# christianhbye/21cmVAE

Measured on AMD Instinct MI355X. Metric: emulated signals/sec (batched predict), higher is better.
Workload: dtype f16 (f32 accumulate)

## Files before the change

21cmvae_amd/_native.py:

```python
import ctypes as C
import os
import threading
import weakref

import numpy as np

HERE = os.path.dirname(os.path.abspath(__file__))
LIB_PATH = os.environ.get("V21_LIB") or os.path.join(HERE, "libv21.so")

PREC_F32, PREC_F16, PREC_BF16 = 0, 1, 2
PRECISIONS = {"f32": PREC_F32, "fp32": PREC_F32, "float32": PREC_F32,
              "f16": PREC_F16, "fp16": PREC_F16, "float16": PREC_F16,
              "bf16": PREC_BF16, "bfloat16": PREC_BF16}
ACT_LINEAR, ACT_RELU, ACT_GAUSS = 0, 1, 2
FWD_IN_TRANSFORM, FWD_OUT_TRANSFORM, FWD_FORCE_GENERIC, FWD_NO_SMALL, FWD_FORCE_CHAIN, FWD_FORCE_JIT = 1, 2, 4, 8, 16, 32
COMM_ID_BYTES = 128


class EngineUnavailable(RuntimeError):
    """libv21.so cannot be loaded or no MI355X is visible."""


class EngineError(RuntimeError):
    """A v21_* call returned a negative status."""
# ... 40 lines not shown


class SampleOut(C.Structure):
    _fields_ = [(k, C.c_void_p) for k in SAMPLE_OUTPUTS]


_P = C.c_void_p
_F = C.POINTER(C.c_float)
SIGNATURES = {
    "v21_last_error": (C.c_char_p, []),
    "v21_version": (C.c_int, []),
    "v21_device_count": (C.c_int, [C.POINTER(C.c_int)]),
    "v21_ctx_create": (C.c_int, [C.c_int, C.POINTER(_P)]),
    "v21_ctx_destroy": (C.c_int, [_P]),
    "v21_ctx_sync": (C.c_int, [_P]),
    "v21_ctx_set_stream": (C.c_int, [_P, _P]),
    "v21_ctx_get_stream": (C.c_int, [_P, C.POINTER(_P)]),
    "v21_malloc": (C.c_int, [_P, C.c_size_t, C.POINTER(_P)]),
    "v21_free": (C.c_int, [_P, _P]),
    "v21_memcpy_h2d": (C.c_int, [_P, _P, _P, C.c_size_t]),
    "v21_memcpy_d2h": (C.c_int, [_P, _P, _P, C.c_size_t]),
    "v21_memset": (C.c_int, [_P, _P, C.c_int, C.c_size_t]),
    "v21_event_create": (C.c_int, [_P, C.POINTER(_P)]),
    "v21_event_destroy": (C.c_int, [_P, _P]),
    "v21_event_record": (C.c_int, [_P, _P]),
    "v21_event_elapsed_ms": (C.c_int, [_P, _P, _P, C.POINTER(C.c_float)]),
    "v21_mlp_create": (C.c_int, [_P, C.c_int, C.POINTER(C.c_int), C.POINTER(C.c_int), C.POINTER(_P)]),
    "v21_mlp_destroy": (C.c_int, [_P]),
    "v21_mlp_num_params": (C.c_int, [_P, C.POINTER(C.c_size_t)]),
    "v21_mlp_set_weights": (C.c_int, [_P, _F, C.c_size_t]),
    "v21_mlp_get_weights": (C.c_int, [_P, _F, C.c_size_t]),
    "v21_mlp_set_input_transform": (C.c_int, [_P, C.POINTER(AffineIn)]),
    "v21_mlp_set_output_transform": (C.c_int, [_P, C.POINTER(AffineOut)]),
    "v21_mlp_has_fused": (C.c_int, [_P, C.c_int, C.POINTER(C.c_int)]),
    "v21_mlp_jit": (C.c_int, [_P, C.c_int, C.c_int, C.POINTER(C.c_int)]),
    "v21_jit_prebuild": (C.c_int, [C.c_int, C.POINTER(C.c_int), C.POINTER(C.c_int), C.c_int, C.c_char_p]),
    "v21_mlp_forward": (C.c_int, [_P, _P, C.c_int, C.c_int64, _F, C.c_int, C.c_int]),
    "v21_mlp_forward_dev": (C.c_int, [_P, _P, C.c_int64, C.c_int64, _P, C.c_int64, C.c_int, C.c_int]),
    "v21_trainer_create": (C.c_int, [_P, C.c_int, C.c_int, C.POINTER(_P)]),
    "v21_trainer_destroy": (C.c_int, [_P]),
    "v21_trainer_set_adam": (C.c_int, [_P, C.POINTER(Adam)]),
    "v21_trainer_set_lr": (C.c_int, [_P, C.c_float]),
    "v21_trainer_get_lr": (C.c_int, [_P, C.POINTER(C.c_float)]),
    "v21_trainer_set_data": (C.c_int, [_P, C.c_int, _F, _F, _F, C.c_int64]),
    "v21_trainer_run_epoch": (C.c_int, [_P, C.POINTER(C.c_int32), C.c_int, C.POINTER(C.c_double)]),
    "v21_trainer_eval": (C.c_int, [_P, C.c_int, C.c_int, C.POINTER(C.c_double)]),
    "v21_trainer_step_dev": (C.c_int, [_P, _P, _P, _P, C.c_int, C.c_int]),
    "v21_trainer_last_step_loss": (C.c_int, [_P, C.POINTER(C.c_double)]),
    "v21_trainer_get_state": (C.c_int, [_P, C.POINTER(C.c_int64), _F, _F, C.c_size_t]),
    "v21_trainer_set_state": (C.c_int, [_P, C.c_int64, _F, _F, C.c_size_t]),
    "v21_trainer_get_grad": (C.c_int, [_P, _F, C.c_size_t]),
    "v21_trainer_use_graph": (C.c_int, [_P, C.c_int]),
    "v21_debug_poison_lds": (C.c_int, [_P, C.c_uint32]),
    "v21_debug_check_chain_jobs": (C.c_int, [_P, C.c_longlong, C.c_longlong]),
    "v21_debug_trainer_counters": (C.c_int, [_P, C.POINTER(C.c_longlong)]),
    "v21_route_forward": (C.c_int, [C.c_int, C.POINTER(C.c_int), C.POINTER(C.c_int), C.c_int, C.c_int64, C.c_int, C.c_int, C.POINTER(C.c_int)]),
    "v21_route_train": (C.c_int, [C.c_int, C.POINTER(C.c_int), C.POINTER(C.c_int), C.c_int, C.c_int, C.c_int, C.c_int, C.c_int,
                                  C.POINTER(C.c_int), C.POINTER(C.c_int)]),
    "v21_trainer_jit": (C.c_int, [_P, C.c_int, C.POINTER(C.c_int)]),
    "v21_mlp_last_route": (C.c_int, [_P, C.POINTER(C.c_int), C.POINTER(C.c_longlong)]),
    "v21_mlp_jacobian": (C.c_int, [_P, _P, C.c_int, C.c_int64, _F, _F, C.c_int, C.c_int]),
    "v21_mlp_jacobian_dev": (C.c_int, [_P, _P, C.c_int64, C.c_int64, _P, C.c_int64, _P, C.c_int, C.c_int]),
    "v21_mlp_set_likelihood": (C.c_int, [_P, _F, _F, C.c_int32]),
    "v21_mlp_loglike": (C.c_int, [_P, _P, C.c_int, C.c_int64, _F, _F, C.c_int, C.c_int]),
    "v21_mlp_loglike_dev": (C.c_int, [_P, _P, C.c_int64, C.c_int64, _P, _P, C.c_int, C.c_int]),
    "v21_route_jacobian": (C.c_int, [C.c_int, C.POINTER(C.c_int), C.POINTER(C.c_int), C.c_int, C.c_int64, C.c_int, C.POINTER(C.c_int)]),
    "v21_mlp_last_jac_route": (C.c_int, [_P, C.POINTER(C.c_int), C.POINTER(C.c_longlong)]),
    "v21_mlp_fisher": (C.c_int, [_P, _P, C.c_int, C.c_int64, _F, _F, _F, C.c_int, C.c_int]),
    "v21_mlp_fisher_dev": (C.c_int, [_P, _P, C.c_int64, C.c_int64, _P, _P, _P, C.c_int, C.c_int]),
    "v21_mlp_fit": (C.c_int, [_P, _P, C.c_int, C.c_int64, _F, C.c_int64, C.POINTER(FitOpts), _P, _F, _F, _F, C.POINTER(C.c_int32),
                              C.c_int, C.c_int]),
    "v21_mlp_fit_dev": (C.c_int, [_P, _P, C.c_int64, C.c_int64, _P, C.c_int64, C.POINTER(FitOpts), _P, _P, _P, _P, _P, C.c_int, C.c_int]),
    "v21_mlp_sample": (C.c_int, [_P, _P, C.c_int, C.c_int64, _F, C.c_int64, C.POINTER(SampleOpts), _P, C.POINTER(SampleOut),
                                 C.c_int, C.c_int]),
    "v21_mlp_sample_dev": (C.c_int, [_P, _P, C.c_int64, C.c_int64, _P, C.c_int64, C.POINTER(SampleOpts), _P, C.POINTER(SampleOut),
                                     C.c_int, C.c_int]),
    "v21_nuisance_whiten": (C.c_int, [C.POINTER(C.c_double), _F, C.c_int32, C.c_int32, C.POINTER(C.c_double), C.POINTER(C.c_double)]),
    "v21_mlp_set_nuisance": (C.c_int, [_P, C.POINTER(C.c_double), C.c_int32, C.c_int32]),
    "v21_mlp_nuisance_info": (C.c_int, [_P, C.POINTER(C.c_int32)]),
    "v21_mlp_nuisance_coef": (C.c_int, [_P, _P, C.c_int, C.c_int64, C.POINTER(C.c_double), C.c_int, C.c_int]),
    "v21_trainer_last_route": (C.c_int, [_P, C.POINTER(C.c_int), C.POINTER(C.c_int), C.POINTER(C.c_longlong), C.POINTER(C.c_longlong)]),
    "v21_route_name": (C.c_char_p, [C.c_int, C.c_int]),
    "v21_trainer_get_data_dev": (C.c_int, [_P, C.c_int, C.POINTER(_P), C.POINTER(_P), C.POINTER(_P), C.POINTER(C.c_int64)]),
    "v21_debug_clock_probe_start": (C.c_int, [_P, C.c_double, C.c_double]),
    "v21_debug_forward_clocked": (C.c_int, [_P, _P, C.c_int64, C.c_int64, _P, C.c_int64, C.c_int, C.c_int, _P]),
    "v21_debug_clock_probe_read": (C.c_int, [_P, C.POINTER(C.c_double), C.POINTER(C.c_double), C.POINTER(C.c_double), C.POINTER(C.c_int)]),
    "v21_trainer_set_vae": (C.c_int, [_P, C.c_float, C.c_int, C.c_uint64]),
    "v21_trainer_enable_stamps": (C.c_int, [_P, C.c_int]),
    "v21_trainer_chain_stamps": (C.c_int, [_P, C.POINTER(C.c_uint64), C.c_int]),
    "v21_host_alloc": (C.c_int, [_P, C.c_size_t, C.POINTER(_P)]),
    "v21_host_free": (C.c_int, [_P, _P]),
    "v21_sweep_create": (C.c_int, [C.POINTER(_P), C.c_int, C.POINTER(_P)]),
    "v21_sweep_destroy": (C.c_int, [_P]),
    "v21_sweep_run_epoch": (C.c_int, [_P, C.POINTER(C.c_int32), C.c_int, C.POINTER(C.c_double)]),
    "v21_joint_create": (C.c_int, [_P, _P, C.c_int, C.POINTER(_P)]),
    "v21_joint_destroy": (C.c_int, [_P]),
    "v21_joint_run_epoch": (C.c_int, [_P, C.POINTER(C.c_int32), C.c_int, C.POINTER(C.c_double)]),
    "v21_joint_eval": (C.c_int, [_P, C.POINTER(C.c_double)]),
    "v21_comm_get_unique_id": (C.c_int, [_P, _P]),
    "v21_comm_init": (C.c_int, [_P, C.c_int, C.c_int, _P]),
    "v21_comm_init_host": (C.c_int, [_P, C.c_int, C.c_int, C.POINTER(CommHostOps)]),
    "v21_comm_destroy": (C.c_int, [_P]),
    "v21_comm_init_null": (C.c_int, [_P, C.c_int, C.c_int]),
    "v21_comm_set_buckets": (C.c_int, [_P, C.c_int]),
    "v21_trainer_phase_timing": (C.c_int, [_P, C.c_int, C.c_int]),
    "v21_trainer_phase_times": (C.c_int, [_P, C.POINTER(C.c_double), C.POINTER(C.c_int)]),
# ... 132 lines not shown
        h, self.h = self.h, None
        try:
            self._destroy(h)
        except Exception:
            pass
        parents, self._parents = self._parents, []
        for p in parents:
            p._children -= 1
            p._try_destroy()

    def __del__(self):
        try:
            if hasattr(self, "_finalized"):
                self._release()
        except Exception:
            pass


class Context:
    _default = {}

    def __init__(self, device=0):
        self.lib = load_library()
        n = C.c_int(0)
        st = self.lib.v21_device_count(C.byref(n))
        if st != 0 or n.value < 1:
            raise EngineUnavailable("no HIP device visible (v21_device_count -> %d, n=%d): the MI355X "
                                    "engine has no CPU fallback" % (st, n.value))
        h = _P()
        check(self.lib.v21_ctx_create(device, C.byref(h)))
        self.h, self.device = h, device
        self.lock = threading.Lock()
        self.nranks, self.rank = 1, 0
        self._host_ops = None
        self._pin_pool = {"free": [], "live": 0, "lock": threading.Lock()}

    @classmethod
    def default(cls, device=None):
        if device is None:
            device = int(os.environ.get("LOCAL_RANK", "0")) if os.environ.get("V21_DEVICE_FROM_RANK") else 0
        if device not in cls._default:
            cls._default[device] = cls(device)
        return cls._default[device]

    def sync(self):
        check(self.lib.v21_ctx_sync(self.h))

    def set_stream(self, hip_stream):
        check(self.lib.v21_ctx_set_stream(self.h, _P(hip_stream)))

    def poison_lds(self, pattern=0xFFFFFFFF):
        check(self.lib.v21_debug_poison_lds(self.h, pattern))

    def clock_probe_start(self, duration_ms, period_us=50.0):
        check(self.lib.v21_debug_clock_probe_start(self.h, float(duration_ms), float(period_us)))

    def clock_probe_read(self):
        a, b, c_, n = C.c_double(0), C.c_double(0), C.c_double(0), C.c_int(0)
        check(self.lib.v21_debug_clock_probe_read(self.h, C.byref(a), C.byref(b), C.byref(c_), C.byref(n)))
        return {"ghz_mean": a.value, "ghz_min": b.value, "ghz_max": c_.value, "samples": n.value}

    def memset(self, dptr, byte, nbytes):
        check(self.lib.v21_memset(self.h, _P(dptr), int(byte), int(nbytes)))

    def malloc(self, nbytes):
        p = _P()
        check(self.lib.v21_malloc(self.h, nbytes, C.byref(p)))
        return p.value

    PIN_MIN_BYTES = 8 << 20
    PIN_POOL_MAX = 4

    def pinned_empty(self, shape, dtype=np.float32):
        nbytes = int(np.prod(shape)) * np.dtype(dtype).itemsize
        if nbytes < self.PIN_MIN_BYTES:
            return None
        pool, ptr = self._pin_pool, None
        with pool["lock"]:
            for i, (p, cap) in enumerate(pool["free"]):
                if cap >= nbytes:
                    ptr, cap_ = pool["free"].pop(i)
                    break
            if ptr is None:
                if pool["live"] + len(pool["free"]) >= self.PIN_POOL_MAX:
                    if pool["free"]:
                        pool["free"].sort(key=lambda t: t[1])
                        q, _ = pool["free"].pop(0)
                        self.lib.v21_host_free(self.h, _P(q))
                    else:
                        return None
                hp = _P()
                if self.lib.v21_host_alloc(self.h, nbytes, C.byref(hp)) != 0:
                    return None
                ptr, cap_ = hp.value, nbytes
            pool["live"] += 1
        raw = (C.c_char * nbytes).from_address(ptr)
        arr = np.frombuffer(raw, dtype=dtype, count=int(np.prod(shape))).reshape(shape)

        def _back(pool=pool, ptr=ptr, cap=cap_):
            with pool["lock"]:
                pool["live"] -= 1
                pool["free"].append((ptr, cap))
        weakref.finalize(raw, _back)
        return arr

    def free(self, dptr):
# ... 586 lines not shown
```

21cmvae_amd/csrc/api_forward.hip:

```cpp
#include "api_internal.h"

namespace v21 {
#define V21_DECL(a)                                                      \
  hipError_t launch_fused_##a##_F32(const FusedArgs&, hipStream_t);      \
  hipError_t launch_fused_##a##_F16x2sp(const FusedArgs&, hipStream_t);  \
  hipError_t launch_fused_##a##_BF16x2sp(const FusedArgs&, hipStream_t);
V21_ARCH_LIST(V21_DECL)
#undef V21_DECL
hipError_t launch_fused_S1_F16x2spClk(const FusedArgs&, hipStream_t);
hipError_t launch_fused_S1_BF16x2spClk(const FusedArgs&, hipStream_t);
}

typedef hipError_t (*fused_launcher)(const FusedArgs&, hipStream_t);
struct FusedEntry {
  int L;
  const int* dims;
  const int* act;
  fused_launcher fn[3];
};
#define V21_ENTRY(a) \
  {Arch##a::L, Arch##a::dims, Arch##a::act, {launch_fused_##a##_F32, launch_fused_##a##_F16x2sp, launch_fused_##a##_BF16x2sp}},
static const FusedEntry g_fused[] = {V21_ARCH_LIST(V21_ENTRY)};
#undef V21_ENTRY

// ... 329 lines not shown
  hipError_t rt = hipSuccess;
  if (route == FWD_FUSED || route == FWD_FUSED_RT) {
    CHK(ensure_stream(m, precision));
    a.x = d_x; a.ldx = ldx; a.y = d_y; a.ldy = ldy; a.n_rows = n;
    a.stream = m->d_stream[precision];
    const bool tout = (flags & V21_FWD_OUT_TRANSFORM) != 0;
    a.out_std = tout ? m->out_std : 1.0f;
    a.out_mean_scale = tout ? 1.0f : 0.0f;
    a.in_transform = (flags & V21_FWD_IN_TRANSFORM) ? 1 : 0;
    if (a.in_transform) a.tin = m->tin;
#ifdef V21_FUSED_STAMP
    a.dbg = (unsigned long long*)(getenv("V21_FUSED_DBG_PTR") ? strtoull(getenv("V21_FUSED_DBG_PTR"), nullptr, 0) : 0ull);
#endif
  }
  if (route == FWD_FUSED_RT) {
    rt = v21::jit_launch(jk, m->ctx->device, a, m->ctx->stream);
    if (rt != hipSuccess) (void)hipGetLastError();
    if (rt != hipSuccess && !force_jit) { q.jit = 0; route = decide_forward(q); }
  }
  note_route(m, route);
  if (route == FWD_TABLE) return forward_chain(m, d_x, ldx, n, d_y, ldy, precision, flags);
  if (route == FWD_GENERIC) return forward_generic(m, d_x, ldx, n, d_y, ldy, precision, flags);
  if (route == FWD_FUSED_RT) {
    if (rt == hipSuccess) return V21_OK;
    std::string why;
    v21::jit_state(jk, &why);
    return fail(V21_ERR_UNSUPPORTED, "V21_FWD_FORCE_JIT: %s (%s)", why.c_str(), hipGetErrorString(rt));
  }
  if (m->clk_stamps) {
    a.dbg = m->clk_stamps;
    HIPCHK((precision == V21_PREC_F16 ? launch_fused_S1_F16x2spClk : launch_fused_S1_BF16x2spClk)(a, m->ctx->stream));
    return V21_OK;
  }
  HIPCHK(g_fused[m->fused_id].fn[precision](a, m->ctx->stream));
  return V21_OK;
}
extern "C" int v21_mlp_forward_dev(v21_mlp* m, const float* d_x, int64_t ldx, int64_t n, float* d_y, int64_t ldy,
                                   int precision, int flags) {
  CHK(fwd_args(m, d_x && d_y, true, n, ldx, ldy, V21_DTYPE_F32, precision, flags));
  return n == 0 ? V21_OK : forward_rows(m, d_x, ldx, n, d_y, ldy, precision, flags);
}
extern "C" int v21_debug_forward_clocked(v21_mlp* m, const float* d_x, int64_t ldx, int64_t n, float* d_y, int64_t ldy, int precision,
                                         int flags, unsigned long long* d_stamps) {
  if (!m || !d_stamps) return fail(V21_ERR_ARG, "null argument");
  if (m->fused_id < 0 || g_fused[m->fused_id].dims != ArchS1::dims || (precision != V21_PREC_F16 && precision != V21_PREC_BF16))
    return fail(V21_ERR_UNSUPPORTED, "clock-stamped kernels exist for the headline stack (archs.h S1) in f16 / bf16 only");
  if (flags & (V21_FWD_FORCE_GENERIC | V21_FWD_FORCE_CHAIN | V21_FWD_FORCE_JIT)) return fail(V21_ERR_ARG, "route flags do not apply");
  m->clk_stamps = d_stamps;
  const int r = v21_mlp_forward_dev(m, d_x, ldx, n, d_y, ldy, precision, flags | V21_FWD_NO_SMALL);
  m->clk_stamps = nullptr;
  return r;
}

extern "C" int v21_mlp_jit(v21_mlp* m, int precision, int wait_ms, int* status) {
  if (!m || !status) return fail(V21_ERR_ARG, "null argument");
  if (precision < 0 || precision > 2) return fail(V21_ERR_ARG, "precision %d unknown", precision);
  *status = -1;
  if (m->fused_id >= 0) { *status = 1; return V21_OK; }
  std::string why;
  if (!v21::jit_eligible(m->L, m->dims.data(), m->act.data(), &why)) return fail(V21_ERR_UNSUPPORTED, "no fused kernel for this stack: %s", why.c_str());
  v21::JitKernel* k = jit_kernel(m, precision);
  if (!k) return fail(V21_ERR_UNSUPPORTED, "run-time compilation is switched off (V21_JIT=0) and no cached kernel exists");
  int s = v21::jit_state(k);
  if (s == v21::JIT_COMPILING && wait_ms != 0) s = v21::jit_wait(k, wait_ms);
  *status = s;
  if (s == v21::JIT_FAILED) {
    v21::jit_state(k, &why);
    return fail(V21_ERR_UNSUPPORTED, "fused kernel of this stack: %s", why.c_str());
  }
  return V21_OK;
}
extern "C" int v21_jit_prebuild(int n_layers, const int* dims, const int* act, int precision, const char* dir) {
  if (!dims || !act) return fail(V21_ERR_ARG, "null argument");
  std::string why;
  if (v21::jit_prebuild(n_layers, dims, act, precision, dir, &why) != 0) return fail(V21_ERR_UNSUPPORTED, "%s", why.c_str());
  return V21_OK;
}

extern "C" int v21_mlp_forward(v21_mlp* m, const void* x, int x_dtype, int64_t n, float* y, int precision, int flags) {
  flags &= 0xFF;
  CHK(fwd_args(m, x && y, false, n, 0, 0, x_dtype, precision, flags));
  if (n == 0) return V21_OK;
  hipStream_t st = m->ctx->stream;
  const int din = m->dims[0], dout = m->dims[m->L];
  const long long chunk = 1 << 18;
  const size_t need = (size_t)std::min<long long>(n, chunk);
  CHK(m->d_xs.reserve(need * din));
  CHK(m->d_xs64.reserve(need * din));
  CHK(m->d_ys.reserve(need * dout));
  std::vector<float> tmp;
  const bool tin = (flags & V21_FWD_IN_TRANSFORM) != 0;
  auto host_value = [&](long long r, int j) -> float {
    const v21_affine_in& a = m->tin;
    if (x_dtype == V21_DTYPE_F64) {
      const double t = ((const double*)x)[r * din + j];
      if (!tin) return (float)t;
      return par_transform_f64(t, a.log_mask[j], a.zero_floor[j], a.lo[j], a.span[j]);
    }
    const float f = ((const float*)x)[r * din + j];
    if (!tin) return f;
    return par_transform_f32(f, a.log_mask[j], a.zero_floor[j], a.lo[j], a.span[j]);
  };
  const FwdQuery hq{m->L, m->dims.data(), m->act.data(), m->fused_id >= 0, 0, precision, (long long)n, flags & ~V21_FWD_IN_TRANSFORM, (long long)dout};
  if (decide_forward(hq) == FWD_SMALL && (!tin || din <= 8)) {
    const long long ldp = p16(din);
    CHK(m->d_xpad.reserve((size_t)(n + 2) * ldp));
// ... 184 lines not shown
```

21cmvae_amd/csrc/fused_fwd.h:

```cpp
#pragma once
#ifndef __HIPCC_RTC__
#include <hip/hip_runtime.h>
#endif

#include <type_traits>
#include <utility>

#include "../../include/v21_types.h"
#include "par_transform.h"

namespace v21 {

typedef float f32x16 __attribute__((ext_vector_type(16)));
typedef float f32x4 __attribute__((ext_vector_type(4)));
typedef _Float16 f16x8 __attribute__((ext_vector_type(8)));
typedef __bf16 bf16x8 __attribute__((ext_vector_type(8)));
typedef unsigned u32x4 __attribute__((ext_vector_type(4)));
typedef short i16x2 __attribute__((ext_vector_type(2)));
typedef float f32x2 __attribute__((ext_vector_type(2)));
typedef _Float16 f16x2 __attribute__((ext_vector_type(2)));
typedef __bf16 bf16x2 __attribute__((ext_vector_type(2)));

constexpr int kFragBytes = 1024;
constexpr int kWaves = 4;
// ... 201 lines not shown
      constexpr int I = decltype(i)::value;
      glds16(g + I * G::WAVES * kFragBytes, voff, s + I * G::WAVES * kFragBytes);
    });
  }
}

template <class G, int B, int I>
__device__ __forceinline__ void issue_piece(const unsigned char* gstream, unsigned char* smem,
                                            int wave, int lane) {
  if constexpr (B >= 0 && B < G::n_blocks()) {
    if constexpr (I < G::blk_glds(B)) {
      const unsigned char* g = gstream + (size_t)B * G::BLK * kFragBytes + I * G::WAVES * kFragBytes;
      const unsigned voff = wave * kFragBytes + lane * 16;
      const unsigned s = lds_addr(smem) + (B % G::RING) * G::BLK * kFragBytes + wave * kFragBytes +
                         I * G::WAVES * kFragBytes;
      glds16(g, voff, s);
    }
  }
}

template <class G, int CT, int D, int S, bool SPREAD>
__device__ __forceinline__ void ring_boundary(const unsigned char* gstream, unsigned char* smem,
                                              int wave, int lane, unsigned long long* g_dbg = nullptr) {
  constexpr int kBlkFrags = G::BLK, kRing = G::RING;
  if constexpr (S % kBlkFrags == 0 && S < G::padded()) {
    constexpr int B = S / kBlkFrags;
    constexpr int last_issued = (B + kRing - 3 > kRing - 1) ? B + kRing - 3 : kRing - 1;
    constexpr int GA = [] {
      int s = 0;
      for (int i = B + 1; i <= last_issued; ++i) s += G::blk_glds(i);
      return s;
    }();
    constexpr int S_issue = (B < kRing) ? 0 : (B - kRing + 2 + (SPREAD ? 1 : 0)) * kBlkFrags;
    constexpr int SA = G::stores_before_step(S, CT, D) - G::stores_before_step(S_issue, CT, D);
    constexpr int N = (GA + SA) > 63 ? 63 : (GA + SA);
#ifdef V21_FUSED_STAMP
    { unsigned long long t; asm volatile("s_memtime %0\n\ts_waitcnt lgkmcnt(0)" : "=s"(t)::"memory");
      ((unsigned long long*)(smem + G::RING * G::BLK * kFragBytes))[wave * 512 + 2 * B] = t; }
#endif
    wait_vmcnt_barrier<N>();
#ifdef V21_FUSED_STAMP
    { unsigned long long t; asm volatile("s_memtime %0\n\ts_waitcnt lgkmcnt(0)" : "=s"(t)::"memory");
      ((unsigned long long*)(smem + G::RING * G::BLK * kFragBytes))[wave * 512 + 2 * B + 1] = t; }
#endif
    if constexpr (B >= 2 && !SPREAD) issue_block<G, B + kRing - 2>(gstream, smem, wave, lane);
  }
}

template <class G, int F> __device__ __forceinline__ const unsigned char* frag_ptr(const unsigned char* smem, int lane) {
  constexpr int B = F / G::BLK;
  return smem + ((B % G::RING) * G::BLK + (F % G::BLK)) * kFragBytes + lane * 16;
}

template <class Arch, class P>
__global__ void __launch_bounds__(64 * P::WAVES, P::WPS) fused_fwd(const FusedArgs a) {
  constexpr int kWaves = P::WAVES;
  constexpr int kBlkFrags = P::BLK, kRing = P::RING, kFusedLds = fused_lds<P>();
  (void)kFusedLds;
  extern __shared__ __attribute__((aligned(16))) unsigned char smem[];
  using G = Geo<Arch, P>;
  using frag = typename P::frag;
  using Item = typename G::Item;
  constexpr int L = G::L, CT = P::CT, EPI = P::EPI, FPI = P::FPI, IPT = G::IPT;
  constexpr int KSM = G::ks_max();
#ifndef V21_FUSED_D
#define V21_FUSED_D 2
#endif
#ifndef V21_FUSED_SPREAD
#define V21_FUSED_SPREAD 0
#endif
  constexpr int D = P::DEPTH;
  constexpr bool SPREAD = (V21_FUSED_SPREAD != 0) || spread_of<P>::value;
  constexpr int TOTAL = G::total();
  constexpr int NOUT = G::dim(L);
  constexpr int NCH = CT * 8;
  static_assert(G::act(L - 1) == 0, "output layer must be linear");
  static_assert(G::nt_of(L - 1) == 1 || G::ks_of(L - 1) > P::DEPTH, "output layer: too few k-steps per tile for the aux double buffer");
  static_assert(D <= kBlkFrags, "read-ahead must stay within one block");

  const int lane = threadIdx.x & 63;
  const int wave = __builtin_amdgcn_readfirstlane(threadIdx.x >> 6);
  const int r = lane & 31, h = lane >> 5;
  unsigned long long clk_t0 = 0, clk_r0 = 0;
  if constexpr (clk_of<P>::value) {
    asm volatile("s_memtime %0\n\ts_memrealtime %1\n\ts_waitcnt lgkmcnt(0)" : "=s"(clk_t0), "=s"(clk_r0)::"memory");
  }
  const long long wg_row0 = (long long)blockIdx.x * (kWaves * CT * 32);
  const long long row0 = wg_row0 + wave * (CT * 32);

  unsigned bufA[CT][KSM][4], bufB[CT][KSM][4];

  {
    constexpr int K0 = G::dim(0);
    static_for<CT>([&](auto ct_) __attribute__((always_inline)) {
      constexpr int ct = decltype(ct_)::value;
      const long long row = row0 + ct * 32 + r;
      const bool ok = row < a.n_rows;
      const float* xr = a.x + (ok ? row : 0) * a.ldx;
      static_for<G::ks_of(0)>([&](auto ks_) __attribute__((always_inline)) {
        constexpr int ks = decltype(ks_)::value;
        float v[EPI];
        static_for<EPI>([&](auto e_) __attribute__((always_inline)) {
          constexpr int e = decltype(e_)::value;
          constexpr int f0 = FPI * ks + 8 * (e >> 2) + (e & 3);
          constexpr int f1 = f0 + 4;
          float t = 0.f;
          if constexpr (f0 < K0) {
            const bool valid = ok && (h == 0 || f1 < K0);
            if (valid) {
              t = xr[f0 + 4 * h];
              if (a.in_transform) {
                constexpr int g1 = f1 < 8 ? f1 : 7;
                constexpr int g0 = f0 < 8 ? f0 : 7;
                const double zf = h ? a.tin.zero_floor[g1] : a.tin.zero_floor[g0];
                const int lm = h ? a.tin.log_mask[g1] : a.tin.log_mask[g0];
                const double lo = h ? a.tin.lo[g1] : a.tin.lo[g0];
                const double sp = h ? a.tin.span[g1] : a.tin.span[g0];
                t = par_transform_f32(t, lm, zf, lo, sp);
              }
            }
          }
          v[e] = t;
        });
#pragma unroll
        for (int wd = 0; wd < 4; ++wd) {
          if constexpr (EPI == 8) bufA[ct][ks][wd] = P::pack2(v[2 * wd], v[2 * wd + 1]);
          else bufA[ct][ks][wd] = __builtin_bit_cast(unsigned, v[wd]);
        }
      });
    });
  }

  static_for<kRing>([&](auto b) __attribute__((always_inline)) {
    issue_block<G, decltype(b)::value>(a.stream, smem, wave, lane);
  });

  long long wg_rows = a.n_rows - wg_row0;
  if (wg_rows > kWaves * CT * 32) wg_rows = kWaves * CT * 32;
  if (wg_rows < 0) wg_rows = 0;
  const unsigned out_bytes = (unsigned)(wg_rows * a.ldy * 4);
  __amdgpu_buffer_rsrc_t orsrc =
      __builtin_amdgcn_make_buffer_rsrc((void*)(a.y + wg_row0 * a.ldy), 0, out_bytes, 0x00020000);
  const unsigned ldy_b = (unsigned)a.ldy * 4u;
  const unsigned ovoff = (unsigned)(wave * (CT * 32) + 4 * h) * ldy_b + (unsigned)r * 4u;

  frag q[D + 1];
  f32x16 auxb[2];
  f32x16 acc[2][CT];

  auto epilogue_chunk = [&](auto g_, auto c_) __attribute__((always_inline)) {
    constexpr int GT = decltype(g_)::value;
    constexpr int c = decltype(c_)::value;
    constexpr Item t = G::tile_at(GT);
    constexpr int l = t.l, nt = t.nt;
    constexpr int ct = c / 8, pr = c % 8;
    if constexpr (l < L - 1) {
      constexpr int item = IPT * nt + (2 * pr) / EPI, e0 = (2 * pr) % EPI;
      if constexpr (item < G::ks_of(l + 1)) {
        auto& out = (l & 1) ? bufA : bufB;
        const float x0 = acc[GT & 1][ct][2 * pr], x1 = acc[GT & 1][ct][2 * pr + 1];
        if constexpr (EPI == 8) {
          unsigned w = P::pack2(x0, x1);
          if constexpr (G::act(l) != 0) {
            const i16x2 z = {0, 0};
            w = __builtin_bit_cast(unsigned, __builtin_elementwise_max(__builtin_bit_cast(i16x2, w), z));
          }
          out[ct][item][e0 / 2] = w;
        } else {
          int b0 = __builtin_bit_cast(int, x0), b1 = __builtin_bit_cast(int, x1);
          if constexpr (G::act(l) != 0) { b0 = max(b0, 0); b1 = max(b1, 0); }
          out[ct][item][e0] = (unsigned)b0;
          out[ct][item][e0 + 1] = (unsigned)b1;
        }
      }
    } else {
      const float obias = auxb[GT & 1][0], omean = auxb[GT & 1][1] * a.out_mean_scale;
      unsigned voff = ovoff + (unsigned)(32 * nt) * 4u;
      if (32 * nt + r >= NOUT) voff = 0xFFFFFFF0u;
#pragma unroll
      for (int u = 0; u < 2; ++u) {
        const int i = 2 * pr + u;
        const unsigned soff = (unsigned)(ct * 32 + (i & 3) + 8 * (i >> 2)) * ldy_b;
        float y;
        if constexpr (EPI == 8) {
          y = __builtin_fmaf(acc[GT & 1][ct][i], a.out_std, __builtin_fmaf(obias, a.out_std, omean));
        } else {
          y = (acc[GT & 1][ct][i] + obias) * a.out_std + omean;
        }
// ... 52 lines not shown
        constexpr int GP = GT > 0 ? GT - 1 : 0;
        constexpr int CPK = G::chunks_per_kstep(GP, NCH);
        constexpr bool whole_first = (GT > 0) && (G::spread_limit(GP) == 0);
        if constexpr (whole_first && it.ks == 0) {
          epilogue_range(std::integral_constant<int, GP>{}, std::integral_constant<int, 0>{},
                         std::integral_constant<int, NCH>{});
        }
#ifdef V21_FUSED_STAMP
        if constexpr (it.ks == 0) {
          unsigned long long t; asm volatile("s_memtime %0\n\ts_waitcnt lgkmcnt(0)" : "=s"(t)::"memory");
          ((unsigned long long*)(smem + kFusedLds))[wave * 512 + 128 + GT] = t; }
#endif
        auto& in = (it.l & 1) ? bufB : bufA;
        const frag w = q[C % (D + 1)];
#pragma unroll
        for (int ct = 0; ct < CT; ++ct) {
          f32x16 c0;
          if constexpr (it.ks == 0) {
            if constexpr (it.l < L - 1) c0 = auxb[GT & 1];
            else
#pragma unroll
              for (int i = 0; i < 16; ++i) c0[i] = 0.f;
          } else {
            c0 = acc[GT & 1][ct];
          }
          acc[GT & 1][ct] = P::template mfma<(it.l == L - 1)>(w, operand(in, ct, it.ks), c0);
        }
        if constexpr (GT > 0 && !whole_first) {
          constexpr int lo = it.ks * CPK < NCH ? it.ks * CPK : NCH;
          constexpr int hi = (it.ks + 1) * CPK < NCH ? (it.ks + 1) * CPK : NCH;
          epilogue_range(std::integral_constant<int, GP>{}, std::integral_constant<int, lo>{},
                         std::integral_constant<int, hi>{});
        }
      }
    }
  });
  epilogue_range(std::integral_constant<int, G::n_tiles() - 1>{}, std::integral_constant<int, 0>{},
                 std::integral_constant<int, NCH>{});
  if constexpr (clk_of<P>::value) {
    unsigned long long t1, r1;
    unsigned xcc, hwid;
    asm volatile("s_memtime %0\n\ts_memrealtime %1\n\ts_getreg_b32 %2, hwreg(HW_REG_XCC_ID)\n\ts_getreg_b32 %3, hwreg(HW_REG_HW_ID)\n\ts_waitcnt lgkmcnt(0)"
                 : "=s"(t1), "=s"(r1), "=s"(xcc), "=s"(hwid)::"memory");
    if (a.dbg && wave == 0 && lane == 0) {
      unsigned long long* gd = a.dbg + (size_t)blockIdx.x * 5;
      gd[0] = clk_t0; gd[1] = clk_r0; gd[2] = t1; gd[3] = r1; gd[4] = (unsigned long long)(xcc & 0xF) | ((unsigned long long)hwid << 8);
    }
  }
#ifdef V21_FUSED_STAMP
  if (a.dbg) {
    unsigned long long t; asm volatile("s_memtime %0\n\ts_waitcnt lgkmcnt(0)" : "=s"(t)::"memory");
    unsigned long long* sd = (unsigned long long*)(smem + kFusedLds) + wave * 512;
    sd[127] = t;
    __builtin_amdgcn_s_waitcnt(0xC07F);
    unsigned long long* gd = a.dbg + ((size_t)blockIdx.x * kWaves + wave) * 512;
#pragma unroll
    for (int k = 0; k < 8; ++k) gd[64 * k + lane] = sd[64 * k + lane];
  }
#endif
}

}
```

21cmvae_amd/csrc/par_transform.h:

```cpp
#pragma once
#ifndef __HIPCC_RTC__
#include <hip/hip_runtime.h>
#endif

#include "../../include/v21_types.h"

namespace v21 {
__host__ __device__ __forceinline__ float par_transform_f32(float x, int lm, double zf, double lo, double span) {
  if (zf > 0.0 && x == 0.f) x = (float)zf;
  double t = (double)x;
  if (lm) t = (double)(float)log10(t);
  t -= lo; t /= span; t *= 2.0; t -= 1.0;
  return (float)t;
}
__host__ __device__ __forceinline__ float par_transform_f64(double t, int lm, double zf, double lo, double span) {
  if (zf > 0.0 && t == 0.0) t = zf;
  if (lm) t = log10(t);
  t -= lo; t /= span; t *= 2.0; t -= 1.0;
  return (float)t;
}
}
```

include/v21.h:

```cpp
#ifndef V21_H
#define V21_H

#include <stddef.h>
#include <stdint.h>

#ifdef __cplusplus
extern "C" {
#endif

typedef struct v21_ctx v21_ctx;
typedef struct v21_mlp v21_mlp;
typedef struct v21_trainer v21_trainer;

enum {
  V21_OK = 0,
  V21_ERR_ARG = -1,
  V21_ERR_HIP = -2,
  V21_ERR_UNSUPPORTED = -3,
  V21_ERR_STATE = -4,
  V21_ERR_COMM = -5
};

enum { V21_PREC_F32 = 0, V21_PREC_F16 = 1, V21_PREC_BF16 = 2 };
enum { V21_ACT_LINEAR = 0, V21_ACT_RELU = 1, V21_ACT_GAUSS = 2 };
// ... 64 lines not shown
int v21_route_jacobian(int n_layers, const int* dims, const int* act, int precision, int64_t n, int flags, int* route);
int v21_mlp_last_jac_route(v21_mlp* mlp, int* route, long long counts[4]);

int v21_mlp_fisher(v21_mlp* mlp, const void* x, int x_dtype, int64_t n, float* fisher, float* lnl, float* grad, int precision, int flags);
int v21_mlp_fisher_dev(v21_mlp* mlp, const float* d_x, int64_t ldx, int64_t n, float* d_fisher, float* d_lnl, float* d_grad,
                       int precision, int flags);
int v21_mlp_fit(v21_mlp* mlp, const void* x0, int x_dtype, int64_t n, const float* data, int64_t n_data, const v21_fit_opts* opts,
                void* x_hat, float* lnl, float* lnl_start, float* fisher, int32_t* status, int precision, int flags);
int v21_mlp_fit_dev(v21_mlp* mlp, const float* d_x0, int64_t ldx, int64_t n, const float* d_data, int64_t n_data,
                    const v21_fit_opts* opts, float* d_x_hat, float* d_lnl, float* d_lnl_start, float* d_fisher, int32_t* d_status,
                    int precision, int flags);

int v21_mlp_sample(v21_mlp* mlp, const void* x0, int x_dtype, int64_t n, const float* data, int64_t n_data, const v21_sample_opts* opts,
                   const double* eps_start, const v21_sample_out* out, int precision, int flags);
int v21_mlp_sample_dev(v21_mlp* mlp, const float* d_x0, int64_t ldx, int64_t n, const float* d_data, int64_t n_data,
                       const v21_sample_opts* opts, const double* d_eps_start, const v21_sample_out* out, int precision, int flags);

int v21_nuisance_whiten(const double* basis, const float* inv_var, int32_t n_modes, int32_t out_dim, double* q, double* r);
int v21_mlp_set_nuisance(v21_mlp* mlp, const double* basis, int32_t n_modes, int32_t out_dim);
int v21_mlp_nuisance_info(v21_mlp* mlp, int32_t* n_modes);
int v21_mlp_nuisance_coef(v21_mlp* mlp, const void* x, int x_dtype, int64_t n, double* coef, int precision, int flags);

typedef struct {
  float lr, beta1, beta2, eps;
} v21_adam;

int v21_trainer_create(v21_mlp* mlp, int precision, int max_batch, v21_trainer** out);
int v21_trainer_destroy(v21_trainer* tr);
int v21_trainer_set_adam(v21_trainer* tr, const v21_adam* cfg);
int v21_trainer_set_lr(v21_trainer* tr, float lr);
int v21_trainer_get_lr(v21_trainer* tr, float* lr);
int v21_trainer_set_data(v21_trainer* tr, int which , const float* x,
                         const float* y, const float* row_weight, int64_t n);
int v21_trainer_run_epoch(v21_trainer* tr, const int32_t* perm, int batch, double* loss);
int v21_trainer_eval(v21_trainer* tr, int which, int batch, double* loss);
int v21_trainer_get_data_dev(v21_trainer* tr, int which, const float** x, const float** y, const float** row_weight, int64_t* n);
int v21_trainer_step_dev(v21_trainer* tr, const float* d_x, const float* d_y,
                         const float* d_row_weight, int n_rows, int global_rows);
int v21_trainer_last_step_loss(v21_trainer* tr, double* loss);
int v21_trainer_get_state(v21_trainer* tr, int64_t* iter, float* m, float* v, size_t n);
int v21_trainer_set_state(v21_trainer* tr, int64_t iter, const float* m, const float* v,
                          size_t n);
int v21_trainer_get_grad(v21_trainer* tr, float* g, size_t n);
typedef struct v21_joint v21_joint;
int v21_joint_create(v21_trainer* ae, v21_trainer* em, int latent_layer, v21_joint** out);
int v21_joint_destroy(v21_joint* j);
int v21_joint_run_epoch(v21_joint* j, const int32_t* perm , int batch, double* losses );
int v21_joint_eval(v21_joint* j, double* losses );
int v21_trainer_use_graph(v21_trainer* tr, int enable);
int v21_debug_poison_lds(v21_ctx* ctx, uint32_t pattern);
int v21_debug_clock_probe_start(v21_ctx* ctx, double duration_ms, double period_us);
int v21_debug_forward_clocked(v21_mlp* mlp, const float* d_x, int64_t ldx, int64_t n, float* d_y, int64_t ldy, int precision,
                              int flags, unsigned long long* d_stamps);
int v21_debug_clock_probe_read(v21_ctx* ctx, double* ghz_mean, double* ghz_min, double* ghz_max, int* samples);
int v21_debug_check_chain_jobs(v21_trainer* tr, long long fw_bytes, long long bw_bytes);
int v21_route_forward(int n_layers, const int* dims, const int* act, int precision, int64_t n, int flags, int rt_ready, int* route);
int v21_route_train(int n_layers, const int* dims, const int* act, int precision, int max_batch, int rows, int nranks, int rt_ready, int* fwd, int* upd);
int v21_mlp_last_route(v21_mlp* mlp, int* route, long long counts[8]);
int v21_trainer_last_route(v21_trainer* tr, int* fwd, int* upd, long long fwd_counts[8], long long upd_counts[8]);
const char* v21_route_name(int kind, int route);
int v21_trainer_phase_timing(v21_trainer* tr, int steps, int cut);
int v21_trainer_phase_times(v21_trainer* tr, double* ms, int* steps);
int v21_debug_trainer_counters(v21_trainer* tr, long long out[4]);
int v21_trainer_enable_stamps(v21_trainer* tr, int enable);
int v21_trainer_chain_stamps(v21_trainer* tr, uint64_t* out, int n);
int v21_trainer_set_vae(v21_trainer* tr, float kl_weight, int sample, uint64_t seed);

typedef struct v21_sweep v21_sweep;
int v21_sweep_create(v21_trainer** trainers, int count, v21_sweep** out);
int v21_sweep_destroy(v21_sweep* sw);
int v21_sweep_run_epoch(v21_sweep* sw, const int32_t* perm, int batch, double* losses);

#define V21_COMM_ID_BYTES 128
typedef struct v21_comm_host_ops {
  void* user;
  int (*allreduce_sum_f32)(void* user, float* buf, size_t n);
  int (*reduce_scatter_sum_f32)(void* user, float* buf, size_t n_per);
  int (*allgather_f32)(void* user, float* buf, size_t n_per);
} v21_comm_host_ops;
int v21_comm_get_unique_id(v21_ctx* ctx, void* id );
int v21_comm_init(v21_ctx* ctx, int nranks, int rank, const void* id);
int v21_comm_init_host(v21_ctx* ctx, int nranks, int rank, const v21_comm_host_ops* ops);
int v21_comm_init_null(v21_ctx* ctx, int nranks, int rank);
int v21_comm_set_buckets(v21_ctx* ctx, int buckets);
int v21_comm_destroy(v21_ctx* ctx);
int v21_comm_set_sharded(v21_ctx* ctx, int on);
int v21_comm_info(v21_ctx* ctx, int* nranks, int* rank, int* transport);
int v21_comm_allreduce_f32(v21_ctx* ctx, float* d_buf, size_t n);
int v21_comm_reduce_scatter_f32(v21_ctx* ctx, float* d_buf, size_t n_per);
int v21_comm_allgather_f32(v21_ctx* ctx, float* d_buf, size_t n_per);

#ifdef __cplusplus
}
#endif
#endif
```

Baseline: 1.232 billion.

## Overlap weight prefetch with input loads and use fast parameter transform

The fused forward kernel now issues the weight-ring prefetch before the first-layer input loads and loads all input values up front, so the global loads overlap. The input parameter transform switches to a fast path that replaces the f64 log10 and division with a polynomial log plus Newton-refined reciprocal. A correctness check falls back to the exact routine when rounding is ambiguous. A debug comparison kernel and clock-stamp hooks are added to validate bit-exactness and profile the kernel head. This costs extra registers for the preloaded inputs.

```diff
diff --git a/21cmvae_amd/_native.py b/21cmvae_amd/_native.py
--- a/21cmvae_amd/_native.py
+++ b/21cmvae_amd/_native.py
@@ -116,6 +116,7 @@
     "v21_trainer_get_grad": (C.c_int, [_P, _F, C.c_size_t]),
     "v21_trainer_use_graph": (C.c_int, [_P, C.c_int]),
     "v21_debug_poison_lds": (C.c_int, [_P, C.c_uint32]),
+    "v21_debug_par_transform_compare": (C.c_int, [_P, _P, C.c_int64, C.c_int, C.c_double, C.c_double, C.c_double, _P]),
     "v21_debug_check_chain_jobs": (C.c_int, [_P, C.c_longlong, C.c_longlong]),
     "v21_debug_trainer_counters": (C.c_int, [_P, C.POINTER(C.c_longlong)]),
     "v21_route_forward": (C.c_int, [C.c_int, C.POINTER(C.c_int), C.POINTER(C.c_int), C.c_int, C.c_int64, C.c_int, C.c_int, C.POINTER(C.c_int)]),
@@ -354,6 +355,9 @@
     def poison_lds(self, pattern=0xFFFFFFFF):
         check(self.lib.v21_debug_poison_lds(self.h, pattern))
 
+    def par_transform_compare(self, d_x, n, log_mask, zero_floor, lo, span, d_counts):
+        check(self.lib.v21_debug_par_transform_compare(self.h, _P(d_x), n, int(log_mask), float(zero_floor), float(lo), float(span), _P(d_counts)))
+
     def clock_probe_start(self, duration_ms, period_us=50.0):
         check(self.lib.v21_debug_clock_probe_start(self.h, float(duration_ms), float(period_us)))
 
diff --git a/21cmvae_amd/csrc/api_forward.hip b/21cmvae_amd/csrc/api_forward.hip
--- a/21cmvae_amd/csrc/api_forward.hip
+++ b/21cmvae_amd/csrc/api_forward.hip
@@ -405,6 +405,32 @@
   return r;
 }
 
+__global__ void __launch_bounds__(256) par_transform_compare_kernel(const float* __restrict__ x, long long n, int lm, double zf,
+                                                                    double lo, double span, unsigned long long* counts) {
+  unsigned long long diff = 0, slow = 0;
+  for (long long i = (long long)blockIdx.x * blockDim.x + threadIdx.x; i < n; i += (long long)gridDim.x * blockDim.x) {
+    int s = 0;
+    const float f = v21::par_transform_f32_fast(x[i], lm, zf, lo, span, &s);
+    const float r = v21::par_transform_f32(x[i], lm, zf, lo, span);
+    diff += __builtin_bit_cast(unsigned, f) != __builtin_bit_cast(unsigned, r);
+    slow += (unsigned)s;
+  }
+  if (diff) atomicAdd(&counts[0], diff);
+  if (slow) atomicAdd(&counts[1], slow);
+}
+extern "C" int v21_debug_par_transform_compare(v21_ctx* c, const float* d_x, int64_t n, int log_mask, double zero_floor, double lo,
+                                               double span, unsigned long long* d_counts) {
+  if (!d_x || !d_counts || n < 0) return fail(V21_ERR_ARG, "bad argument");
+  CHK(use(c));
+  HIPCHK(hipMemsetAsync(d_counts, 0, 2 * sizeof(unsigned long long), c->stream));
+  if (n == 0) return V21_OK;
+  const long long blocks = (n + 255) / 256;
+  hipLaunchKernelGGL(par_transform_compare_kernel, dim3((unsigned)(blocks < 4096 ? blocks : 4096)), dim3(256), 0, c->stream, d_x,
+                     (long long)n, log_mask, zero_floor, lo, span, d_counts);
+  HIPCHK(hipGetLastError());
+  return V21_OK;
+}
+
 extern "C" int v21_mlp_jit(v21_mlp* m, int precision, int wait_ms, int* status) {
   if (!m || !status) return fail(V21_ERR_ARG, "null argument");
   if (precision < 0 || precision > 2) return fail(V21_ERR_ARG, "precision %d unknown", precision);
diff --git a/21cmvae_amd/csrc/fused_fwd.h b/21cmvae_amd/csrc/fused_fwd.h
--- a/21cmvae_amd/csrc/fused_fwd.h
+++ b/21cmvae_amd/csrc/fused_fwd.h
@@ -277,6 +277,18 @@
   return smem + ((B % G::RING) * G::BLK + (F % G::BLK)) * kFragBytes + lane * 16;
 }
 
+#ifdef V21_FUSED_STAMP
+#define V21_HEAD_STAMP(k, drain)                                                                   \
+  {                                                                                                \
+    unsigned long long t_;                                                                         \
+    if (drain) asm volatile("s_waitcnt vmcnt(0)" ::: "memory");                                    \
+    asm volatile("s_memtime %0\n\ts_waitcnt lgkmcnt(0)" : "=s"(t_)::"memory");                     \
+    ((unsigned long long*)(smem + kFusedLds))[wave * 512 + 200 + (k)] = t_;                        \
+  }
+#else
+#define V21_HEAD_STAMP(k, drain)
+#endif
+
 template <class Arch, class P>
 __global__ void __launch_bounds__(64 * P::WAVES, P::WPS) fused_fwd(const FusedArgs a) {
   constexpr int kWaves = P::WAVES;
@@ -315,13 +327,34 @@
 
   unsigned bufA[CT][KSM][4], bufB[CT][KSM][4];
 
+  V21_HEAD_STAMP(0, false)
+  static_for<kRing>([&](auto b) __attribute__((always_inline)) {
+    issue_block<G, decltype(b)::value>(a.stream, smem, wave, lane);
+  });
+  V21_HEAD_STAMP(3, false)
+
   {
     constexpr int K0 = G::dim(0);
+    float xv[CT][G::ks_of(0)][EPI];
     static_for<CT>([&](auto ct_) __attribute__((always_inline)) {
       constexpr int ct = decltype(ct_)::value;
       const long long row = row0 + ct * 32 + r;
-      const bool ok = row < a.n_rows;
-      const float* xr = a.x + (ok ? row : 0) * a.ldx;
+      const float* xr = a.x + (row < a.n_rows ? row : 0) * a.ldx;
+      static_for<G::ks_of(0)>([&](auto ks_) __attribute__((always_inline)) {
+        constexpr int ks = decltype(ks_)::value;
+        static_for<EPI>([&](auto e_) __attribute__((always_inline)) {
+          constexpr int e = decltype(e_)::value;
+          constexpr int f0 = FPI * ks + 8 * (e >> 2) + (e & 3);
+          constexpr int f1 = f0 + 4;
+          if constexpr (f0 < K0) xv[ct][ks][e] = xr[f1 < K0 ? f0 + 4 * h : f0];
+          else xv[ct][ks][e] = 0.f;
+        });
+      });
+    });
+    V21_HEAD_STAMP(1, true)
+    static_for<CT>([&](auto ct_) __attribute__((always_inline)) {
+      constexpr int ct = decltype(ct_)::value;
+      const bool ok = row0 + ct * 32 + r < a.n_rows;
       static_for<G::ks_of(0)>([&](auto ks_) __attribute__((always_inline)) {
         constexpr int ks = decltype(ks_)::value;
         float v[EPI];
@@ -333,7 +366,7 @@
           if constexpr (f0 < K0) {
             const bool valid = ok && (h == 0 || f1 < K0);
             if (valid) {
-              t = xr[f0 + 4 * h];
+              t = xv[ct][ks][e];
               if (a.in_transform) {
                 constexpr int g1 = f1 < 8 ? f1 : 7;
                 constexpr int g0 = f0 < 8 ? f0 : 7;
@@ -341,7 +374,7 @@
                 const int lm = h ? a.tin.log_mask[g1] : a.tin.log_mask[g0];
                 const double lo = h ? a.tin.lo[g1] : a.tin.lo[g0];
                 const double sp = h ? a.tin.span[g1] : a.tin.span[g0];
-                t = par_transform_f32(t, lm, zf, lo, sp);
+                t = par_transform_f32_fast(t, lm, zf, lo, sp);
               }
             }
           }
@@ -354,11 +387,8 @@
         }
       });
     });
-  }
-
-  static_for<kRing>([&](auto b) __attribute__((always_inline)) {
-    issue_block<G, decltype(b)::value>(a.stream, smem, wave, lane);
-  });
+    V21_HEAD_STAMP(2, false)
+  }
 
   long long wg_rows = a.n_rows - wg_row0;
   if (wg_rows > kWaves * CT * 32) wg_rows = kWaves * CT * 32;
@@ -517,6 +547,7 @@
     unsigned long long t; asm volatile("s_memtime %0\n\ts_waitcnt lgkmcnt(0)" : "=s"(t)::"memory");
     unsigned long long* sd = (unsigned long long*)(smem + kFusedLds) + wave * 512;
     sd[127] = t;
+    { unsigned hwid_; asm volatile("s_getreg_b32 %0, hwreg(HW_REG_HW_ID)" : "=s"(hwid_)); sd[206] = hwid_; }
     __builtin_amdgcn_s_waitcnt(0xC07F);
     unsigned long long* gd = a.dbg + ((size_t)blockIdx.x * kWaves + wave) * 512;
 #pragma unroll
diff --git a/21cmvae_amd/csrc/par_transform.h b/21cmvae_amd/csrc/par_transform.h
--- a/21cmvae_amd/csrc/par_transform.h
+++ b/21cmvae_amd/csrc/par_transform.h
@@ -19,4 +19,61 @@
   t -= lo; t /= span; t *= 2.0; t -= 1.0;
   return (float)t;
 }
+
+__host__ __device__ __forceinline__ double pt_rcp_seed(double d) {
+#if defined(__HIP_DEVICE_COMPILE__)
+  return (double)__builtin_amdgcn_rcpf((float)d);
+#else
+  return (double)(1.0f / (float)d);
+#endif
 }
+__host__ __device__ __forceinline__ double pt_div_approx(double n, double d) {
+  double r = pt_rcp_seed(d);
+  const double e = __builtin_fma(-d, r, 1.0);
+  r = __builtin_fma(r, e, r);
+  const double q = n * r;
+  const double rem = __builtin_fma(-q, d, n);
+  return __builtin_fma(rem, r, q);
+}
+__host__ __device__ __forceinline__ float par_transform_f32_fast(float x0, int lm, double zf, double lo, double span,
+                                                                 int* slow_path = nullptr) {
+  float x = x0;
+  if (zf > 0.0 && x == 0.f) x = (float)zf;
+  double t = (double)x;
+  const double aspan = __builtin_fabs(span);
+  bool ok = aspan >= 0x1p-100 && aspan <= 0x1p100;
+  if (lm) {
+    const unsigned u = __builtin_bit_cast(unsigned, x);
+    ok = ok && u >= 0x00800000u && u <= 0x7F7FFFFFu;
+    unsigned mb = (u & 0x007FFFFFu) | 0x3F800000u;
+    int k = (int)(u >> 23) - 127;
+    if (mb >= 0x3FB504F3u) { mb -= 0x00800000u; k += 1; }
+    const double m = (double)__builtin_bit_cast(float, mb);
+    const double s = pt_div_approx(m - 1.0, m + 1.0);
+    const double z = s * s;
+    double p = 0x1.da5d89f186bcbp-5;
+    p = __builtin_fma(p, z, 0x1.11ac1e5a1c809p-4);
+    p = __builtin_fma(p, z, 0x1.436e526a7ec67p-4);
+    p = __builtin_fma(p, z, 0x1.8b4df2f3f047ep-4);
+    p = __builtin_fma(p, z, 0x1.fc3fa615105c7p-4);
+    p = __builtin_fma(p, z, 0x1.63c62775250d8p-3);
+    p = __builtin_fma(p, z, 0x1.287a7636f435fp-2);
+    p = __builtin_fma(p, z, 0x1.bcb7b1526e50ep-1);
+    const double y = __builtin_fma(s, p, (double)k * 0x1.34413509f79ffp-2);
+    const float ya = (float)(y * (1.0 - 0x1p-40)), yb = (float)(y * (1.0 + 0x1p-40));
+    ok = ok && ya == yb;
+    t = (double)ya;
+  }
+  t -= lo;
+  const double q = pt_div_approx(t, span);
+  const double rem = __builtin_fma(-q, span, t);
+  const unsigned long long qb = __builtin_bit_cast(unsigned long long, q);
+  const unsigned long long qe = (qb >> 52) & 0x7FFull;
+  const double half_ulp = __builtin_bit_cast(double, (qe > 300 ? qe - 53 : 0ull) << 52);
+  ok = ok && (rem == 0.0 || (qe > 300 && qe < 0x7FFull && (qb & 0xFFFFFFFFFFFFFull) != 0 && __builtin_fabs(rem) < aspan * half_ulp));
+  const double w = __builtin_fma(q, 2.0, -1.0);
+  if (slow_path) *slow_path = ok ? 0 : 1;
+  if (!ok) return par_transform_f32(x0, lm, zf, lo, span);
+  return (float)w;
+}
+}
diff --git a/include/v21.h b/include/v21.h
--- a/include/v21.h
+++ b/include/v21.h
@@ -140,6 +140,8 @@
 int v21_debug_clock_probe_start(v21_ctx* ctx, double duration_ms, double period_us);
 int v21_debug_forward_clocked(v21_mlp* mlp, const float* d_x, int64_t ldx, int64_t n, float* d_y, int64_t ldy, int precision,
                               int flags, unsigned long long* d_stamps);
+int v21_debug_par_transform_compare(v21_ctx* ctx, const float* d_x, int64_t n, int log_mask, double zero_floor, double lo,
+                                    double span, unsigned long long* d_counts);
 int v21_debug_clock_probe_read(v21_ctx* ctx, double* ghz_mean, double* ghz_min, double* ghz_max, int* samples);
 int v21_debug_check_chain_jobs(v21_trainer* tr, long long fw_bytes, long long bw_bytes);
 int v21_route_forward(int n_layers, const int* dims, const int* act, int precision, int64_t n, int flags, int rt_ready, int* route);
```

Result: no change. 1.224 billion (-0.6%).

## Overlap input staging with first weight block fetch and add fast log10 path

Applied to the files above, without the earlier changes.

The input-row loads and parameter transform now overlap with the first weight-block issue. When the first layer has a single k-step, raw inputs are loaded before the issue, and the transform and packing run after a waitcnt. The remaining ring blocks are issued only after that. The double-precision library log10 is replaced with a polynomial log10 that falls back to the library call when the f32 rounding may be ambiguous, so results stay correctly rounded. The cost is more registers for the staged inputs and delaying the later ring blocks behind the head.

```diff
diff --git a/21cmvae_amd/csrc/fused_fwd.h b/21cmvae_amd/csrc/fused_fwd.h
--- a/21cmvae_amd/csrc/fused_fwd.h
+++ b/21cmvae_amd/csrc/fused_fwd.h
@@ -288,14 +288,8 @@
   using Item = typename G::Item;
   constexpr int L = G::L, CT = P::CT, EPI = P::EPI, FPI = P::FPI, IPT = G::IPT;
   constexpr int KSM = G::ks_max();
-#ifndef V21_FUSED_D
-#define V21_FUSED_D 2
-#endif
-#ifndef V21_FUSED_SPREAD
-#define V21_FUSED_SPREAD 0
-#endif
   constexpr int D = P::DEPTH;
-  constexpr bool SPREAD = (V21_FUSED_SPREAD != 0) || spread_of<P>::value;
+  constexpr bool SPREAD = spread_of<P>::value;
   constexpr int TOTAL = G::total();
   constexpr int NOUT = G::dim(L);
   constexpr int NCH = CT * 8;
@@ -315,8 +309,11 @@
 
   unsigned bufA[CT][KSM][4], bufB[CT][KSM][4];
 
-  {
-    constexpr int K0 = G::dim(0);
+  constexpr int K0 = G::dim(0);
+  constexpr bool kStageX = G::ks_of(0) == 1;
+  float xraw[CT][EPI];
+  auto head = [&](auto phase_) __attribute__((always_inline)) {
+    constexpr int PH = decltype(phase_)::value;
     static_for<CT>([&](auto ct_) __attribute__((always_inline)) {
       constexpr int ct = decltype(ct_)::value;
       const long long row = row0 + ct * 32 + r;
@@ -333,31 +330,41 @@
           if constexpr (f0 < K0) {
             const bool valid = ok && (h == 0 || f1 < K0);
             if (valid) {
-              t = xr[f0 + 4 * h];
-              if (a.in_transform) {
-                constexpr int g1 = f1 < 8 ? f1 : 7;
-                constexpr int g0 = f0 < 8 ? f0 : 7;
-                const double zf = h ? a.tin.zero_floor[g1] : a.tin.zero_floor[g0];
-                const int lm = h ? a.tin.log_mask[g1] : a.tin.log_mask[g0];
-                const double lo = h ? a.tin.lo[g1] : a.tin.lo[g0];
-                const double sp = h ? a.tin.span[g1] : a.tin.span[g0];
-                t = par_transform_f32(t, lm, zf, lo, sp);
+              if constexpr (PH == 2) t = xraw[ct][e];
+              else t = xr[f0 + 4 * h];
+              if constexpr (PH != 1) {
+                if (a.in_transform) {
+                  constexpr int g1 = f1 < 8 ? f1 : 7;
+                  constexpr int g0 = f0 < 8 ? f0 : 7;
+                  const double zf = h ? a.tin.zero_floor[g1] : a.tin.zero_floor[g0];
+                  const int lm = h ? a.tin.log_mask[g1] : a.tin.log_mask[g0];
+                  const double lo = h ? a.tin.lo[g1] : a.tin.lo[g0];
+                  const double sp = h ? a.tin.span[g1] : a.tin.span[g0];
+                  t = par_transform_f32(t, lm, zf, lo, sp);
+                }
               }
             }
           }
+          if constexpr (PH == 1) xraw[ct][e] = t;
           v[e] = t;
         });
-#pragma unroll
-        for (int wd = 0; wd < 4; ++wd) {
-          if constexpr (EPI == 8) bufA[ct][ks][wd] = P::pack2(v[2 * wd], v[2 * wd + 1]);
-          else bufA[ct][ks][wd] = __builtin_bit_cast(unsigned, v[wd]);
+        if constexpr (PH != 1) {
+#pragma unroll
+          for (int wd = 0; wd < 4; ++wd) {
+            if constexpr (EPI == 8) bufA[ct][ks][wd] = P::pack2(v[2 * wd], v[2 * wd + 1]);
+            else bufA[ct][ks][wd] = __builtin_bit_cast(unsigned, v[wd]);
+          }
         }
       });
     });
-  }
-
-  static_for<kRing>([&](auto b) __attribute__((always_inline)) {
-    issue_block<G, decltype(b)::value>(a.stream, smem, wave, lane);
+  };
+  if constexpr (kStageX) head(std::integral_constant<int, 1>{});
+  issue_block<G, 0>(a.stream, smem, wave, lane);
+  if constexpr (!kStageX) head(std::integral_constant<int, 0>{});
+  __builtin_amdgcn_s_waitcnt(0x0F70);
+  if constexpr (kStageX) head(std::integral_constant<int, 2>{});
+  static_for<kRing - 1>([&](auto b) __attribute__((always_inline)) {
+    issue_block<G, decltype(b)::value + 1>(a.stream, smem, wave, lane);
   });
 
   long long wg_rows = a.n_rows - wg_row0;
diff --git a/21cmvae_amd/csrc/par_transform.h b/21cmvae_amd/csrc/par_transform.h
--- a/21cmvae_amd/csrc/par_transform.h
+++ b/21cmvae_amd/csrc/par_transform.h
@@ -6,10 +6,43 @@
 #include "../../include/v21_types.h"
 
 namespace v21 {
+__host__ __device__ __forceinline__ double log10_fast_f64(double t) {
+  const unsigned long long b = __builtin_bit_cast(unsigned long long, t);
+  unsigned hi = (unsigned)(b >> 32) + (0x3ff00000u - 0x3fe6a09eu);
+  const int k = (int)(hi >> 20) - 0x3ff;
+  hi = (hi & 0x000fffffu) + 0x3fe6a09eu;
+  const double m = __builtin_bit_cast(double, ((unsigned long long)hi << 32) | (b & 0xffffffffull));
+  const double s = (m - 1.0) / (m + 1.0);
+  const double z = s * s;
+  double p = 1.0 / 17.0;
+  p = __builtin_fma(p, z, 1.0 / 15.0);
+  p = __builtin_fma(p, z, 1.0 / 13.0);
+  p = __builtin_fma(p, z, 1.0 / 11.0);
+  p = __builtin_fma(p, z, 1.0 / 9.0);
+  p = __builtin_fma(p, z, 1.0 / 7.0);
+  p = __builtin_fma(p, z, 1.0 / 5.0);
+  p = __builtin_fma(p, z, 1.0 / 3.0);
+  const double r = __builtin_fma(s, p * z, s);
+  return __builtin_fma((double)k, 0.30102999566398119521 , r * 0.86858896380650365530 );
+}
+__host__ __device__ __forceinline__ bool log10_f32_decided(double v) {
+  const unsigned low = (unsigned)__builtin_bit_cast(unsigned long long, v) & 0x1fffffffu;
+  return low - (0x10000000u - 0x1000u) >= 0x2000u;
+}
+__host__ __device__ __attribute__((noinline)) inline float log10_f32_library(double t) { return (float)log10(t); }
+__host__ __device__ __forceinline__ float log10_f32(float x) {
+  const double t = (double)x;
+  if (x > 0.f && x <= 3.40282346638528859812e38f) {
+    const double v = log10_fast_f64(t);
+    if (__builtin_expect(log10_f32_decided(v), 1)) return (float)v;
+  }
+  return log10_f32_library(t);
+}
+
 __host__ __device__ __forceinline__ float par_transform_f32(float x, int lm, double zf, double lo, double span) {
   if (zf > 0.0 && x == 0.f) x = (float)zf;
   double t = (double)x;
-  if (lm) t = (double)(float)log10(t);
+  if (lm) t = (double)log10_f32(x);
   t -= lo; t /= span; t *= 2.0; t -= 1.0;
   return (float)t;
 }
```

Result: no change. 1.189 billion before, 1.198 billion after, median of 6 (+0.8%).
